# stefanopini/simple-HRNet

Measured on AMD Instinct MI355X. Metric: person-crops/sec HRNet-W48 384x288 (model forward + heat-map decode), higher is better.
Workload: dtype bf16; 1 GPU; HRNet-W48 384x288, batch=256 random crops per GPU, bf16 MFMA (BASELINE configs[2]); global_batch=256, micro_batch=256, lanes_per_gpu=1, parallelism=dp1 (crop sharding, RCCL all-gather of keypoints), weights=random-init seeded (synth_state_dict seed 0), BN stats randomised, engine_switches=

## Files before the change

include/hrnet_mi355.h:

```cpp
#ifndef HRNET_MI355_H
#define HRNET_MI355_H

#include <stddef.h>
#include <stdint.h>

#ifdef __cplusplus
extern "C" {
#endif

typedef struct hrn_ctx *hrn_handle;

enum { HRN_F32 = 0, HRN_BF16 = 1, HRN_F16 = 2 };
enum { HRN_BOX_I32 = 0, HRN_BOX_F32 = 1 };
enum { HRN_T_F32 = 0, HRN_T_I64 = 1 };

typedef struct {
    const char *name;
    const void *data;
    int32_t ndim;
    int64_t dims[4];
    int32_t dtype;
} hrn_tensor_desc;

typedef struct {
// ... 167 lines not shown
                        float *pts_dev, float *heatmaps_dev, void *stream);
int hrn_refine_coords(hrn_handle h, const float *heatmaps_dev, int n, int refine, float *coords_dev, void *stream);

int hrn_nms(int32_t *keep_out, int32_t *num_out, const float *boxes_host, int boxes_num, int boxes_dim,
            float nms_overlap_thresh, int device_id);
int hrn_nms_release(int device_id);
const char *hrn_nms_last_error(void);

int hrn_oks_nms(int32_t *keep_out, int32_t *num_out, const double *kpts, const double *areas, const int32_t *order, int n, int J,
                double thresh, const double *sigmas, double in_vis_thre);
int hrn_soft_oks_nms(int32_t *keep_out, int32_t *num_out, const double *kpts, const double *areas, const double *scores_sorted,
                     const int32_t *order, int n, int J, double thresh, const double *sigmas, double in_vis_thre);
int hrn_pose_similarity(const double *boxes_a, const float *poses_a, int na, const double *boxes_b, const float *poses_b, int nb, int J,
                        float *sim_bbox, float *sim_pose);
int hrn_assignment(const double *cost, int rows, int cols, int32_t *row_to_col);

typedef struct {
    char name[96];
    int32_t c, h, w;
    int32_t conv_index;
} hrn_tap_info;
int hrn_tap_count(hrn_handle h);
int hrn_get_tap_info(hrn_handle h, int index, hrn_tap_info *out);
int hrn_forward_tap(hrn_handle h, const void *images_dev, int n, const char *tap_name, int crop0, int ncrops, int crop_step,
                    float *dst_dev, float *heatmaps_dev, void *stream);

int hrn_conv_count(hrn_handle h);
int hrn_get_conv_info(hrn_handle h, int index, hrn_conv_info *out);
double hrn_flops_per_crop(hrn_handle h);
int64_t hrn_workspace_bytes(hrn_handle h);
int64_t hrn_map_rebuilds(hrn_handle h);
int hrn_launches_per_pass(hrn_handle h);
int hrn_stem_fused(hrn_handle h);
int hrn_conv_compact(hrn_handle h, int index);
const char *hrn_switches(hrn_handle h);
int64_t hrn_debug_pad_violations(hrn_handle h);
int hrn_plan_block_map(hrn_handle h, int group, int n, int reverse, int32_t *blocks, int capacity, int32_t *members,
                       int member_capacity);
int hrn_plan_direct_map(hrn_handle h, int group, int n, int32_t *blocks, int capacity, int32_t *members, int member_capacity,
                        int32_t *pixels_per_tile);
int hrn_plan_s2_map(hrn_handle h, int group, int n, int32_t *blocks, int capacity, int32_t *parts, int part_capacity,
                    int32_t *active);
int hrn_profile_pass(hrn_handle h, const void *images_dev, int n, float *conv_ms, int conv_ms_len,
                     float *other_ms , void *stream);
const char *hrn_version(void);

#ifdef __cplusplus
}
#endif
#endif
```

simple-hrnet_amd/_lib.py:

```python
from __future__ import annotations

import ctypes
import os
import shutil
import subprocess
from typing import List

_HERE = os.path.dirname(os.path.abspath(__file__))
CSRC = os.path.join(_HERE, "csrc")
INCLUDE = os.path.join(os.path.dirname(_HERE), "include")
LIB_PATH = os.path.join(_HERE, "libhrnet_mi355.so")
if os.environ.get("HRN_LIB_TAG"):
    LIB_PATH = LIB_PATH.replace(".so", "_%s.so" % os.environ["HRN_LIB_TAG"])
SOURCES = ["kernels.hip", "conv3x3_lds.hip", "conv_s2.hip", "stem_fused.hip", "conv3x3_f32.hip", "bottleneck_chain.hip", "prepath.hip", "warp.hip", "nms.hip", "postproc.cpp", "hrnet_mi355.cpp",
           "decode.hip",
           "score.hip",
           "draw.hip",
           "track.hip",
           "pose_nms.hip",
           "letterbox.hip",
           "assoc.hip",
           "conv3x3_lds_f16.hip", "conv_s2_f16.hip", "bottleneck_chain_f16.hip"]
HEADERS = [os.path.join(CSRC, "kernels.h"), os.path.join(CSRC, "dt16.h"), os.path.join(CSRC, "argmax.h"), os.path.join(CSRC, "conv3x3_n96.inc"), os.path.join(CSRC, "conv3x3_lds.inc"),
           os.path.join(CSRC, "conv_s2.inc"), os.path.join(CSRC, "bottleneck_chain.inc"), os.path.join(INCLUDE, "hrnet_mi355.h")]
# ... 207 lines not shown
    "hrn_yuv_from_bgr": (ctypes.c_int, [ctypes.c_int, ctypes.c_int, _P, ctypes.c_int, _P]),
    "hrn_crop_geometry": (ctypes.c_int, [_P, ctypes.c_int, ctypes.c_int, _P, ctypes.c_int, ctypes.c_int, ctypes.c_int, ctypes.c_int, _P, _P]),
    "hrn_crop_geometry_last_error": (ctypes.c_char_p, []),
    "hrn_pose_boxes": (ctypes.c_int, [_P, ctypes.c_int, ctypes.c_int, _P, ctypes.c_int, ctypes.c_float, ctypes.c_int, ctypes.c_double,
                                      ctypes.c_double, _P]),
    "hrn_pose_boxes_last_error": (ctypes.c_char_p, []),
    "hrn_boxes_from_poses": (ctypes.c_int, [_P, _P, ctypes.c_int, ctypes.c_int, _P, ctypes.c_int, ctypes.c_float, ctypes.c_int,
                                            ctypes.c_double, ctypes.c_double, _P, _P]),
    "hrn_preprocess_frames_dev": (ctypes.c_int, [_P, ctypes.POINTER(Frame), ctypes.c_int, _P, ctypes.c_int, _P, ctypes.c_int, ctypes.c_int,
                                                 _P, _P, _P, _P]),
    "hrn_preprocess_frames_yuv_dev": (ctypes.c_int, [_P, ctypes.POINTER(YuvFrameC), ctypes.c_int, _P, ctypes.c_int, _P, ctypes.c_int,
                                                     ctypes.c_int, _P, _P, _P, _P]),
    "hrn_forward_flip_tta": (ctypes.c_int, [_P, _P, ctypes.c_int, _P, ctypes.c_int, ctypes.c_int, _P, _P, _P, _P]),
    "hrn_forward_refined": (ctypes.c_int, [_P, _P, ctypes.c_int, _P, ctypes.c_int, ctypes.c_int, _P, _P, _P]),
    "hrn_refine_coords": (ctypes.c_int, [_P, _P, ctypes.c_int, ctypes.c_int, _P, _P]),
    "hrn_nms": (ctypes.c_int, [_P, _P, _P, ctypes.c_int, ctypes.c_int, ctypes.c_float, ctypes.c_int]),
    "hrn_nms_release": (ctypes.c_int, [ctypes.c_int]),
    "hrn_nms_last_error": (ctypes.c_char_p, []),
    "hrn_oks_nms": (ctypes.c_int, [_P, _P, _P, _P, _P, ctypes.c_int, ctypes.c_int, ctypes.c_double, _P, ctypes.c_double]),
    "hrn_soft_oks_nms": (ctypes.c_int, [_P, _P, _P, _P, _P, _P, ctypes.c_int, ctypes.c_int, ctypes.c_double, _P, ctypes.c_double]),
    "hrn_pose_similarity": (ctypes.c_int, [_P, _P, ctypes.c_int, _P, _P, ctypes.c_int, ctypes.c_int, _P, _P]),
    "hrn_assignment": (ctypes.c_int, [_P, ctypes.c_int, ctypes.c_int, _P]),
    "hrn_tap_count": (ctypes.c_int, [_P]),
    "hrn_get_tap_info": (ctypes.c_int, [_P, ctypes.c_int, ctypes.POINTER(TapInfo)]),
    "hrn_forward_tap": (ctypes.c_int, [_P, _P, ctypes.c_int, ctypes.c_char_p, ctypes.c_int, ctypes.c_int, ctypes.c_int, _P, _P, _P]),
    "hrn_conv_count": (ctypes.c_int, [_P]),
    "hrn_get_conv_info": (ctypes.c_int, [_P, ctypes.c_int, ctypes.POINTER(ConvInfo)]),
    "hrn_flops_per_crop": (ctypes.c_double, [_P]),
    "hrn_workspace_bytes": (ctypes.c_int64, [_P]),
    "hrn_map_rebuilds": (ctypes.c_int64, [_P]),
    "hrn_launches_per_pass": (ctypes.c_int, [_P]),
    "hrn_switches": (ctypes.c_char_p, [_P]),
    "hrn_stem_fused": (ctypes.c_int, [_P]),
    "hrn_conv_compact": (ctypes.c_int, [_P, ctypes.c_int]),
    "hrn_debug_pad_violations": (ctypes.c_int64, [_P]),
    "hrn_plan_block_map": (ctypes.c_int, [_P, ctypes.c_int, ctypes.c_int, ctypes.c_int, _P, ctypes.c_int, _P, ctypes.c_int]),
    "hrn_plan_direct_map": (ctypes.c_int, [_P, ctypes.c_int, ctypes.c_int, _P, ctypes.c_int, _P, ctypes.c_int, _P]),
    "hrn_plan_s2_map": (ctypes.c_int, [_P, ctypes.c_int, ctypes.c_int, _P, ctypes.c_int, _P, ctypes.c_int, _P]),
    "hrn_profile_pass": (ctypes.c_int, [_P, _P, ctypes.c_int, ctypes.POINTER(ctypes.c_float), ctypes.c_int,
                                        ctypes.POINTER(ctypes.c_float), _P]),
    "hrn_version": (ctypes.c_char_p, []),
}

_lib = None


def load(auto_build: bool = True) -> ctypes.CDLL:
    global _lib
    if _lib is not None:
        return _lib
    if auto_build and needs_build():
        build()
    lib = ctypes.CDLL(LIB_PATH)
    for name, (res, args) in SYMBOLS.items():
        fn = getattr(lib, name)
        fn.restype = res
        fn.argtypes = args
    _lib = lib
    return lib


def header_symbols() -> List[str]:
    import re

    text = open(os.path.join(INCLUDE, "hrnet_mi355.h")).read()
    text = re.sub(r"/\*.*?\*/", "", text, flags=re.S)
# ... 2 lines not shown
```

simple-hrnet_amd/csrc/ctx_plan.inc:

```
    int new_tensor(int ch, int h, int w) {
        Tensor t;
        t.c = ch, t.h = h, t.w = w, t.wp = w + 1, t.hp = h + 1, t.hpwp = t.wp * t.hp;
        for (size_t i = 0; i < buffers.size(); ++i)
            if (!buffers[i].in_use && buffers[i].c == ch && buffers[i].h == h && buffers[i].w == w) {
                t.buf = (int)i;
                break;
            }
        if (t.buf < 0) {
            Buffer b;
            b.c = ch, b.h = h, b.w = w;
            b.lead_rows = (size_t)t.wp + 1;
            b.rows = b.lead_rows + (size_t)max_batch * t.hpwp + t.wp + 1 + kConvBlockRows;
            b.bytes = (size_t)align_up((int64_t)(b.rows * ch * esize), 256);
            buffers.push_back(b);
            t.buf = (int)buffers.size() - 1;
        }
        buffers[t.buf].in_use = true;
        tensors.push_back(t);
        return (int)tensors.size() - 1;
    }
    void release(int t) { buffers[tensors[t].buf].in_use = false; }

    int default_nr(int cout, int stride) const {
        int nr = (cout % 64 == 0) ? 4 : (cout % 48 == 0) ? 3 : 2;
// ... 371 lines not shown
        if (is16() && !disable_stem_fuse && !disable_stem_mfma && stem_fused_fits(tensors[x].wp, W)) {
            stem_fuse = true;
            convs.back().w2_image = true;
            stemf = S2Group();
            stemf.conv_idx = {(int)convs.size() - 1};
            for (int t = 0; t < 2; ++t) {
                if (stemf.probs.empty()) {
                    stemf.probs.push_back(S2Group::Prob());
                    stemf.probs[0].in_t = stem_out_t;
                    stemf.probs[0].rows = 1, stemf.probs[0].tiles_per_image = tensors[x].h;
                }
                stemf.probs[0].parts.push_back({(int)convs.size() - 1, t});
            }
        }
        release(stem_out_t);
        char buf[96];
        x = add_layer1(x, 4);
        std::vector<int> xs;
        xs.push_back(add_conv("transition1.0.0", "transition1.0.1", x, c, 3, 1, 1, -1, false));
        xs.push_back(add_conv("transition1.1.0.0", "transition1.1.0.1", x, 2 * c, 3, 2, 1, -1, false));
        emit_convs({(int)convs.size() - 2, (int)convs.size() - 1});
        release(x);
        add_stage("stage2.0", xs, 2);
        xs.push_back(add_conv("transition2.2.0.0", "transition2.2.0.1", xs[1], 4 * c, 3, 2, 1));
        for (int m = 0; m < 4; ++m) {
            snprintf(buf, sizeof buf, "stage3.%d", m);
            add_stage(buf, xs, 3);
        }
        xs.push_back(add_conv("transition3.3.0.0", "transition3.3.0.1", xs[2], 8 * c, 3, 2, 1));
        add_stage("stage4.0", xs, 4);
        add_stage("stage4.1", xs, 4);
        add_stage("stage4.2", xs, 1);
        head_in_t = xs[0];
        ops.push_back({OP_HEAD, 0});
        ops.push_back({OP_DECODE, 0});

        layout_blob();
    }

    void index_taps() {
        taps.clear();
        auto add = [&](const std::string &name, int tensor, int op, int conv) {
            for (TapPoint &t : taps)
                if (t.name == name) {
                    t.op = op;
                    return;
                }
            taps.push_back(TapPoint{name, tensor, op, conv});
        };
        for (size_t oi = 0; oi < ops.size(); ++oi) {
            const Op &op = ops[oi];
            switch (op.kind) {
                case OP_STEM:
                case OP_STEM7: add("stem", stem_out_t, (int)oi, -1); break;
                case OP_MAXPOOL: add("maxpool", pool_out_t, (int)oi, -1); break;
                case OP_CONV: add(convs[op.idx].conv, convs[op.idx].out_t, (int)oi, op.idx); break;
                case OP_CONV3_GROUP:
                    for (int ci : groups[op.idx].conv_idx) add(convs[ci].conv, convs[ci].out_t, (int)oi, ci);
                    break;
                case OP_CONV_GROUP:
                    for (int ci : dgroups[op.idx].conv_idx) add(convs[ci].conv, convs[ci].out_t, (int)oi, ci);
                    break;
                case OP_S2_GROUP:
                    for (int ci : s2groups[op.idx].conv_idx) add(convs[ci].conv, convs[ci].out_t, (int)oi, ci);
                    break;
                case OP_CHAIN:
// ... 43 lines not shown
```

simple-hrnet_amd/csrc/ctx_run.inc:

```
    struct Timing {
        std::vector<hipEvent_t> ev;
    };

    bool run_pass(const float *images, int nb, const void *boxes, int box_dtype, float *pts, float *heatmaps,
                  hipStream_t s, Timing *tm, int flip = 0, const TapReq *tap = nullptr, int refine = RF_NONE) {
        if (tm && !hip_ok(hipEventRecord(tm->ev[0], s), "hipEventRecord")) return false;
        const bool fused_stem = stem_fuse && !(tap && tap->op == 0);
        for (size_t oi = 0; oi < ops.size(); ++oi) {
            const bool rev = alternate && (oi & 1);
            hipError_t e = hipSuccess;
            if (fused_stem && oi == 0)
                e = exec_stem_fused(images, nb, s, flip);
            else if (!(fused_stem && (int)oi == stem_conv2_op))
                e = exec_op(ops[oi], rev, images, nb, boxes, box_dtype, pts, heatmaps, s, flip, refine);
            if (!hip_ok(e, "kernel launch")) return false;
            if (tap && tap->op == (int)oi) {
                const Tensor &t = tensors[tap->tensor];
                TapArgs a;
                a.in = row0(tap->tensor), a.dst = tap->dst;
                a.c = t.c, a.h = t.h, a.w = t.w, a.wp = t.wp, a.hpwp = t.hpwp;
                a.crop0 = tap->crop0, a.ncrops = tap->ncrops, a.crop_step = tap->crop_step;
                if (!hip_ok(launch_tap(dtype, a, s), "tap launch")) return false;
            }
            if (tm && !hip_ok(hipEventRecord(tm->ev[oi + 1], s), "hipEventRecord")) return false;
        }
        return true;
    }

    hipError_t exec_stem_fused(const float *images, int nb, hipStream_t s, int flip) {
        S2Group &g = stemf;
        bool hit;
        MapSlot *sl = find_slot(g.slot, nb, &hit);
        hipError_t e = slot_ready(sl, hit, s);
        if (e != hipSuccess) return e;
        if (!hit) {
            sl->nblocks = s2_blocks(g, nb, &g.map_host);
            if (sl->nblocks > g.map_capacity) return hipErrorInvalidValue;
            memcpy(sl->pin, g.map_host.data(), (size_t)sl->nblocks * sizeof(int2));
            e = hipMemcpyAsync(sl->dev, sl->pin, (size_t)sl->nblocks * sizeof(int2), hipMemcpyHostToDevice, s);
            if (e == hipSuccess) e = hipEventRecord(sl->landed, s);
            if (e != hipSuccess) return e;
            sl->nb = nb;
            ++map_builds;
        }
        const Tensor &t = tensors[stem_out_t];
        StemArgs a;
        a.images = images, a.out = nullptr;
        a.w = nullptr, a.bias = (const float *)(blob + stem_b_off), a.wp = (const void *)(blob + stem_wp_off);
        a.n = nb, a.H = H, a.W = W;
        a.out_h = t.h, a.out_w = t.w, a.out_wp = t.wp, a.out_hpwp = t.hpwp;
        a.flip = flip;
        return launch_stem_fused(dtype, s2probs_dev + g.prob_first, sl->dev, sl->nblocks, a, s);
    }

    hipError_t exec_op(const Op &op, bool rev, const float *images, int nb, const void *boxes, int box_dtype, float *pts,
                       float *heatmaps, hipStream_t s, int flip, int refine) {
        hipError_t e = hipSuccess;
        switch (op.kind) {
        case OP_STEM: {
            const Tensor &t = tensors[stem_out_t];
            StemArgs a;
            a.images = images, a.out = row0(stem_out_t);
            a.w = (const float *)(blob + stem_w_off), a.bias = (const float *)(blob + stem_b_off);
            a.wp = (is16() && !disable_stem_mfma) ? (const void *)(blob + stem_wp_off) : nullptr;
            a.n = nb, a.H = H, a.W = W;
            a.out_h = t.h, a.out_w = t.w, a.out_wp = t.wp, a.out_hpwp = t.hpwp;
            a.flip = flip;
            e = launch_stem(dtype, a, s);
            break;
        }
        case OP_STEM7: {
            const Tensor &t = tensors[stem_out_t];
            Stem7Args a;
            a.images = images, a.out = row0(stem_out_t);
            a.w = (const float *)(blob + stem_w_off), a.bias = (const float *)(blob + stem_b_off);
            a.wp = (is16() && !disable_stem_mfma) ? (const void *)(blob + stem_wp_off) : nullptr;
            a.n = nb, a.H = H, a.W = W;
            a.out_h = t.h, a.out_w = t.w, a.out_wp = t.wp, a.out_hpwp = t.hpwp;
            a.flip = flip;
            e = launch_stem7(dtype, a, s);
            break;
        }
        case OP_MAXPOOL: {
            const Tensor &ti = tensors[pool_in_t], &to = tensors[pool_out_t];
            PoolArgs a;
            a.in = row0(pool_in_t), a.out = row0(pool_out_t);
            a.c = to.c, a.n = nb, a.in_wp = ti.wp, a.in_hpwp = ti.hpwp;
            a.out_h = to.h, a.out_w = to.w, a.out_wp = to.wp, a.out_hpwp = to.hpwp;
            e = launch_maxpool(dtype, a, s);
// ... 114 lines not shown
            a.m = nb * to.hpwp, a.h = to.h, a.w = to.w, a.wp = to.wp, a.hpwp = to.hpwp, a.rev = rev, a.max_blocks = chain_blocks;
            e = dtype == HRN_F16 ? launch_bottleneck_chain_f16(a, s) : launch_bottleneck_chain(a, s);
            break;
        }
        case OP_FUSE: {
            FuseGroupArgs ga;
            ga.nf = fuses[op.idx].group;
            for (int k = 0; k < ga.nf; ++k) {
                const FuseOp &f = fuses[op.idx + k];
                const Tensor &to = tensors[f.out_t];
                FuseArgs &a = ga.f[k];
                a.nterms = f.nterms;
                for (int i = 0; i < f.nterms; ++i) {
                    const Tensor &tt = tensors[f.term_t[i]];
                    a.t[i].ptr = row0(f.term_t[i]), a.t[i].shift = f.shift[i];
                    a.t[i].wp = tt.wp, a.t[i].hpwp = tt.hpwp;
                }
                for (int i = f.nterms; i < 4; ++i) a.t[i] = FuseTerm{nullptr, 0, 0, 0};
                a.out = row0(f.out_t), a.c = to.c, a.h = to.h, a.w = to.w, a.wp = to.wp, a.hpwp = to.hpwp;
                a.m = nb * to.hpwp, a.rev = rev;
            }
            e = ga.nf == 1 ? launch_fuse(dtype, ga.f[0], s) : launch_fuse_group(dtype, ga, s);
            break;
        }
        case OP_HEAD: {
            const Tensor &t = tensors[head_in_t];
            HeadArgs a;
            a.in = row0(head_in_t);
            a.wgt = (const float *)(blob + head_w_off), a.bias = (const float *)(blob + head_b_off);
            a.wimg = (is16() && !disable_head_mfma) ? (const void *)(blob + head_wp_off) : nullptr;
            a.heatmaps = heatmaps, a.part_val = part_val, a.part_idx = part_idx;
            a.n = nb, a.c = t.c, a.joints = joints, a.h = t.h, a.w = t.w, a.wp = t.wp, a.hpwp = t.hpwp;
            a.slabs = head_slabs_for(nb), a.slab_px = head_px_for(nb);
            e = launch_head(dtype, a, s);
            break;
        }
        case OP_DECODE: {
            if (!pts) break;
            const Tensor &t = tensors[head_in_t];
            DecodeArgs a{};
            a.part_val = part_val, a.part_idx = part_idx, a.heatmaps = heatmaps, a.boxes = boxes;
            a.box_is_float = box_dtype == HRN_BOX_F32, a.pts = pts;
            a.n = nb, a.joints = joints, a.h = t.h, a.w = t.w, a.slabs = head_slabs_for(nb), a.mode = refine;
            e = launch_decode(a, s);
            break;
        }
    }
        return e;
    }

    bool check_forward_args(const void *images, int n, const void *boxes, float *pts, float *heatmaps, bool outputs_optional = false) {
        if (refuse_plan_only()) return false;
        if (!weights_loaded) {
            err = "weights not loaded (call hrn_load_weights or hrn_adopt_weights)";
            return false;
        }
        if (n < 0 || (n > 0 && !images)) {
            err = "bad images / n";
            return false;
        }
        if (!pts && !heatmaps && !outputs_optional) {
            err = "both pts and heatmaps are NULL";
            return false;
        }
        if (pts && !boxes && n > 0) {
            err = "pts requested without boxes";
// ... 5 lines not shown
```

simple-hrnet_amd/csrc/hrnet_mi355.cpp:

```cpp
#include "../../include/hrnet_mi355.h"

#include <hip/hip_runtime.h>

#include <algorithm>
#include <cmath>
#include <cstdio>
#include <cstdlib>
#include <cstring>
#include <map>
#include <memory>
#include <string>
#include <vector>

#include "assoc_math.h"
#include "letterbox_math.h"
#include "pose_nms_math.h"
#include "kernels.h"
#include "track_geometry.h"

namespace {
#include "ctx_types.h"
}

namespace {
// ... 52 lines not shown
    int small_keep_above = env_sw("HRN_SMALL_KEEP") ? atoi(env_sw("HRN_SMALL_KEEP")) : 300;
    bool disable_chain_ds = env_sw("HRN_DISABLE_CHAIN_DS") != nullptr;
    int pre_mode = env_sw("HRN_PRE_MODE") ? atoi(env_sw("HRN_PRE_MODE")) : 1;
    int chain_blocks = env_sw("HRN_CHAIN_BLOCKS") ? atoi(env_sw("HRN_CHAIN_BLOCKS")) : 512;
    bool disable_chain3 = env_sw("HRN_DISABLE_CHAIN3") != nullptr;
    bool direct_wlds = !(env_sw("HRN_DIRECT_WLDS") && atoi(env_sw("HRN_DIRECT_WLDS")) == 0);
    bool direct_xlds = !(env_sw("HRN_DIRECT_XLDS") && atoi(env_sw("HRN_DIRECT_XLDS")) == 0);
    bool conv_xl(const ConvOp &cv) const {
        return direct_xlds && direct_wlds && is16() && cv.k == 3 && cv.stride == 2 && cv.cin % 32 == 0 && !cv.up && cv.res_t < 0 && cv.nr == 6 &&
               cv.kchunks >= 4;
    }
    bool disable_bbf = env_sw("HRN_BBF") && atoi(env_sw("HRN_BBF")) == 0;
    int bbf_tpb_div = env_sw("HRN_BBF_TPB_DIV") ? std::max(1, atoi(env_sw("HRN_BBF_TPB_DIV"))) : 3;
    double bbf_slide_cost = env_sw("HRN_BBF_SLIDE_COST") ? atof(env_sw("HRN_BBF_SLIDE_COST")) : 24600.0;
    int bbf_min_tiles = env_sw("HRN_BBF_MIN_TILES") ? atoi(env_sw("HRN_BBF_MIN_TILES")) : 1100;
    int dgroup_nr_mode = env_sw("HRN_DGROUP_NR") ? atoi(env_sw("HRN_DGROUP_NR")) : 1;
    bool disable_lds32 = env_sw("HRN_DISABLE_LDS32") != nullptr;
    bool disable_n96 = env_sw("HRN_DISABLE_N96") != nullptr;
    bool disable_fgroup = env_sw("HRN_DISABLE_FGROUP") != nullptr;
    bool disable_f32lds = env_sw("HRN_DISABLE_F32LDS") != nullptr;
    int f32_small_slices = env_sw("HRN_F32_SMALL_SLICES") ? atoi(env_sw("HRN_F32_SMALL_SLICES")) : 0;
    std::vector<Conv3Problem> probs_host;
    bool disable_compact = env_sw("HRN_DISABLE_COMPACT") != nullptr;
    double compact_min_pad = env_sw("HRN_COMPACT_MIN_PAD") ? atof(env_sw("HRN_COMPACT_MIN_PAD")) : 0.08;
    bool disable_s2 = env_sw("HRN_DISABLE_S2") != nullptr;
    int s2_min_tiles = env_sw("HRN_S2_MIN_TILES") ? atoi(env_sw("HRN_S2_MIN_TILES")) : 256;
    int s2_target_blocks = env_sw("HRN_S2_BLOCKS") ? std::max(1, atoi(env_sw("HRN_S2_BLOCKS"))) : 256;
    bool disable_stem_mfma = env_sw("HRN_DISABLE_STEM_MFMA") != nullptr;
    bool disable_stem_fuse = env_sw("HRN_DISABLE_STEM_FUSE") != nullptr;
    bool stem_fuse = false;
    int stem_conv2_op = -1;
    S2Group stemf;
    bool disable_head_mfma = env_sw("HRN_DISABLE_HEAD_MFMA") != nullptr;
    bool direct_nr6 = env_sw("HRN_DIRECT_NR6") ? atoi(env_sw("HRN_DIRECT_NR6")) != 0 : true;
    int half_stages_per_block = env_sw("HRN_HALF_STAGES") ? atoi(env_sw("HRN_HALF_STAGES")) : 8;
    bool alternate = env_sw("HRN_ALTERNATE") ? atoi(env_sw("HRN_ALTERNATE")) != 0 : true;
    int block_order = env_sw("HRN_BLOCK_ORDER") ? atoi(env_sw("HRN_BLOCK_ORDER")) : 1;
    int long_factor = env_sw("HRN_LONG_FACTOR") ? atoi(env_sw("HRN_LONG_FACTOR")) : 4;
    double long_share = env_sw("HRN_LONG_SHARE") ? atof(env_sw("HRN_LONG_SHARE")) : 0.85;
    int head_slabs = 1, head_slab_px = 1024;
    static constexpr int kHeadSlabPxSmall = 256;
    int head_slabs_small = 1;
    int head_px_for(int nb) const { return (long)nb * head_slabs >= 192 ? head_slab_px : kHeadSlabPxSmall; }
    int head_slabs_for(int nb) const { return (long)nb * head_slabs >= 192 ? head_slabs : head_slabs_small; }
    float *part_val = nullptr;
    int *part_idx = nullptr;
    uint64_t map_clock = 0;
    int64_t map_builds = 0;
    float *scratch_hm = nullptr;
    float *scratch_heatmaps() {
        if (!scratch_hm && !hip_ok(hipMalloc((void **)&scratch_hm, (size_t)max_batch * joints * (H / 4) * (W / 4) * sizeof(float)),
                                   "hipMalloc(scratch heat-maps)"))
            scratch_hm = nullptr;
        return scratch_hm;
    }
    int64_t workspace_bytes = 0;

#include "ctx_plan.inc"
#include "ctx_memory.inc"
#include "ctx_weights.inc"
#include "ctx_run.inc"
#include "ctx_scratch.inc"
};

namespace {
using CallScope = hrn_ctx::CallScope;
// ... 1224 lines not shown
    if (!h->run_pass((const float *)images_dev, n, nullptr, 0, nullptr, heatmaps_dev, (hipStream_t)stream, nullptr, 0, &req)) return 8;
    return scope.leave() ? 0 : 6;
}

int hrn_conv_count(hrn_handle h) { return h ? (int)h->convs.size() : 0; }

int hrn_get_conv_info(hrn_handle h, int index, hrn_conv_info *out) {
    if (!h || !out || index < 0 || index >= (int)h->convs.size()) return 1;
    const ConvOp &cv = h->convs[index];
    memset(out, 0, sizeof *out);
    snprintf(out->name, sizeof out->name, "%s", cv.conv.c_str());
    out->cin = cv.cin, out->cout = cv.cout, out->ksize = cv.k, out->stride = cv.stride, out->relu = cv.relu;
    out->has_residual = cv.res_t >= 0;
    out->in_h = h->tensors[cv.in_t].h, out->in_w = h->tensors[cv.in_t].w;
    out->out_h = h->tensors[cv.out_t].h, out->out_w = h->tensors[cv.out_t].w;
    out->kpad = cv.kpad, out->nr = cv.nr, out->algo = cv.fuse_with >= 0 || cv.fused_away ? 2 : cv.n96 ? 3 : cv.s2 ? 4 : cv.algo, out->ks = cv.ks;
    out->w_offset = cv.w_off, out->w_bytes = cv.w_bytes, out->b_offset = cv.b_off;
    out->flops = cv.flops;
    return 0;
}

double hrn_flops_per_crop(hrn_handle h) {
    if (!h) return 0;
    double f = 2.0 * 64 * (h->model == 1 ? 147 : 27) * (h->H / 2) * (double)(h->W / 2);
    for (auto &cv : h->convs) f += cv.flops;
    f += 2.0 * h->joints * h->head_c * (h->H / 4) * (double)(h->W / 4);
    return f;
}

int64_t hrn_workspace_bytes(hrn_handle h) { return h ? h->workspace_bytes : 0; }
int64_t hrn_map_rebuilds(hrn_handle h) { return h ? h->map_builds : -1; }
int hrn_launches_per_pass(hrn_handle h) { return h ? (int)h->ops.size() - (h->stem_fuse ? 1 : 0) : 0; }
int hrn_stem_fused(hrn_handle h) { return h && h->stem_fuse ? 1 : 0; }
int hrn_conv_compact(hrn_handle h, int index) { return h && index >= 0 && index < (int)h->convs.size() && h->convs[index].compact ? 1 : 0; }
const char *hrn_switches(hrn_handle h) { return h ? h->switches.c_str() : ""; }

int64_t hrn_debug_pad_violations(hrn_handle h) {
    if (!h || h->plan_only) return -1;
    if (!h->hip_ok(hipSetDevice(h->device), "hipSetDevice")) return -1;
    unsigned long long *cnt = nullptr, host = 0;
    if (!h->hip_ok(hipMalloc((void **)&cnt, sizeof *cnt), "hipMalloc") || !h->hip_ok(hipMemset(cnt, 0, sizeof *cnt), "hipMemset")) return -1;
    bool ok = h->hip_ok(hipDeviceSynchronize(), "hipDeviceSynchronize");
    for (const Buffer &b : h->buffers) {
        if (!ok) break;
        PadCheckArgs a;
        a.buf = b.dev, a.count = cnt, a.rows = (long)b.rows, a.lead_rows = (long)b.lead_rows;
        a.c = b.c, a.h = b.h, a.w = b.w, a.wp = b.w + 1, a.hpwp = (b.h + 1) * (b.w + 1), a.nmax = h->max_batch;
        ok = h->hip_ok(launch_pad_check(h->dtype, a, nullptr), "pad check launch");
    }
    ok = ok && h->hip_ok(hipMemcpy(&host, cnt, sizeof host, hipMemcpyDeviceToHost), "hipMemcpy");
    (void)hipFree(cnt);
    return ok ? (int64_t)host : -1;
}

int hrn_plan_block_map(hrn_handle h, int group, int n, int reverse, int32_t *blocks, int capacity, int32_t *members, int member_capacity) {
    if (!h || n <= 0 || n > h->max_batch) return -1;
    if (group < 0 || group >= (int)h->groups.size()) return -1;
    const Conv3Group &g = h->groups[group];
    std::vector<int2> map;
    std::vector<int> px;
    const int nblocks = h->group_blocks(g, n, &map, reverse != 0, false, &px);
    for (int i = 0; i < nblocks && i < capacity; ++i) {
        const int x = map[i].x, y = map[i].y;
        int32_t *o = blocks + (size_t)i * 6;
        o[0] = x & 0xff, o[1] = (x >> 8) & 0xff, o[2] = x >> 16, o[3] = y & 0x1fffffff, o[4] = px[i],
        o[5] = ((y >> 29) & 1) | (((y >> 30) & 1) << 1);
// ... 123 lines not shown
```

simple-hrnet_amd/csrc/kernels.h:

```cpp
#pragma once
#include <hip/hip_runtime.h>
#include <stdint.h>

#include <atomic>
#include <cstdlib>
#include <cstring>

namespace hrn {

inline hipError_t set_dynamic_lds(const void *func, int bytes, std::atomic<unsigned long long> &done) {
    int dev = 0;
    hipError_t e = hipGetDevice(&dev);
    if (e != hipSuccess) return e;
    const unsigned long long bit = 1ull << (dev & 63);
    if (done.load(std::memory_order_acquire) & bit) return hipSuccess;
    e = hipFuncSetAttribute(func, hipFuncAttributeMaxDynamicSharedMemorySize, bytes);
    if (e == hipSuccess) done.fetch_or(bit, std::memory_order_release);
    return e;
}

inline const char *hrn_env(const char *name) {
    static const bool debug = [] {
        const char *v = getenv("HRN_DEBUG_ENV");
        return v && *v && strcmp(v, "0") != 0;
// ... 179 lines not shown
hipError_t launch_maxpool(int dtype, const PoolArgs &a, hipStream_t s);

struct FuseTerm {
    const void *ptr;
    int shift;
    int wp, hpwp;
};
struct FuseArgs {
    FuseTerm t[4];
    int nterms;
    void *out;
    int c, h, w, wp, hpwp;
    int m;
    int rev;
};

struct FuseGroupArgs {
    FuseArgs f[4];
    int nf;
    int block_end[4];
};
hipError_t launch_fuse_group(int dtype, FuseGroupArgs &g, hipStream_t s);

constexpr int kMaxJoints = 256;
struct HeadArgs {
    const void *in;
    const float *wgt;
    const void *wimg;
    const float *bias;
    float *heatmaps;
    float *part_val;
    int *part_idx;
    int n, c, joints, h, w, wp, hpwp, slabs, slab_px;
};

enum { RF_NONE = 0, RF_QUARTER = 1, RF_DARK = 2 };
struct DecodeArgs {
    const float *part_val;
    const int *part_idx;
    const void *boxes;
    int box_is_float;
    float *pts;
    int n, joints, h, w, slabs, mode;
    const float *heatmaps;
    float *coords;
};
hipError_t launch_decode(const DecodeArgs &a, hipStream_t s);
hipError_t launch_refine_coords(const DecodeArgs &a, hipStream_t s);

struct TtaArgs {
    float *hm;
    const float *hm_flipped;
    float *preds;
    float *maxvals;
    int pair[kMaxJoints];
    int n, joints, h, w, post_processing;
};
hipError_t launch_tta_decode(const TtaArgs &a, hipStream_t s);

struct ScoreJoint {
    int mu_x, mu_y;
    float weight;
    int draw;
};
struct ScoreArgs {
    const float *heatmaps;
// ... 169 lines not shown
```

simple-hrnet_amd/csrc/kernels.hip:

```cpp
#include "kernels.h"
#include "argmax.h"
#include "dt16.h"
#include <stdlib.h>

namespace hrn {

typedef __attribute__((ext_vector_type(8))) __bf16 bf16x8;
typedef __attribute__((ext_vector_type(8))) short s16x8;
typedef __attribute__((ext_vector_type(4))) short s16x4;
typedef __attribute__((ext_vector_type(4))) float f32x4;

__device__ __forceinline__ float bf16_to_f32(unsigned short h) { return __uint_as_float(((unsigned)h) << 16); }
__device__ __forceinline__ unsigned short f32_to_bf16(float f) {
    unsigned u = __float_as_uint(f);
    u += 0x7fffu + ((u >> 16) & 1u);
    return (unsigned short)(u >> 16);
}

constexpr bool is16(int dt) { return dt != DT_F32; }

template <int DT>
struct Tr;
template <>
struct Tr<DT_BF16> {
    using elem = unsigned short;
    using vec = s16x8;
    using out4 = s16x4;
    static constexpr int KC = 32, VEC = 8;
    static __device__ __forceinline__ float ld(elem e) { return bf16_to_f32(e); }
    static __device__ __forceinline__ elem st(float f) { return f32_to_bf16(f); }
};
template <>
struct Tr<DT_F16> {
    using elem = unsigned short;
    using vec = s16x8;
// ... 771 lines not shown
        }
    }
}

hipError_t launch_stem(int dtype, const StemArgs &a, hipStream_t s) {
    const int m = a.n * a.out_hpwp;
    if (m <= 0) return hipSuccess;
    dim3 grid((m + 255) / 256);
    if (dtype == DT_BF16 && a.wp)
        hipLaunchKernelGGL(stem_mfma_kernel<DT_BF16>, grid, dim3(256), 0, s, a);
    else if (dtype == DT_F16 && a.wp)
        hipLaunchKernelGGL(stem_mfma_kernel<DT_F16>, grid, dim3(256), 0, s, a);
    else if (dtype == DT_BF16)
        hipLaunchKernelGGL(stem_kernel<DT_BF16>, grid, dim3(256), 0, s, a);
    else if (dtype == DT_F16)
        hipLaunchKernelGGL(stem_kernel<DT_F16>, grid, dim3(256), 0, s, a);
    else
        hipLaunchKernelGGL(stem_kernel<DT_F32>, grid, dim3(256), 0, s, a);
    return hipGetLastError();
}

template <int DT>
__device__ __forceinline__ void fuse_body(const FuseArgs &p, const long block, const long nblocks) {
    using T = Tr<DT>;
    using vec = typename T::vec;
    const int cvn = p.c / T::VEC;
    const long bid = p.rev ? nblocks - 1 - block : block;
    const long idx = bid * 256 + threadIdx.x;
    const long total = (long)p.m * cvn;
    if (idx >= total) return;
    const int q = (int)(idx / cvn), cv = (int)(idx - (long)q * cvn);
    const int n = q / p.hpwp, rem = q - n * p.hpwp;
    const int r = rem / p.wp, c = rem - r * p.wp;
    float sum[T::VEC];
#pragma unroll
    for (int t = 0; t < 4; ++t) {
        if (t >= p.nterms) break;
        const FuseTerm ft = p.t[t];
        const long row = ft.shift == 0 ? (long)q : (long)n * ft.hpwp + (long)(r >> ft.shift) * ft.wp + (c >> ft.shift);
        const vec v = *(const vec *)((const typename T::elem *)ft.ptr + row * p.c + cv * T::VEC);
#pragma unroll
        for (int e = 0; e < T::VEC; ++e) {
            const float f = T::ld((typename T::elem)v[e]);
            sum[e] = (t == 0) ? f : sum[e] + f;
        }
    }
    vec o;
#pragma unroll
    for (int e = 0; e < T::VEC; ++e) o[e] = T::st(fmaxf(sum[e], 0.f));
    *(vec *)((typename T::elem *)p.out + (long)q * p.c + cv * T::VEC) = o;
}

template <int DT>
__global__ __launch_bounds__(256) void fuse_kernel(const FuseArgs p) {
    fuse_body<DT>(p, blockIdx.x, gridDim.x);
}

template <int DT>
__global__ __launch_bounds__(256) void fuse_group_kernel(const FuseGroupArgs g) {
    int k = 0;
    long first = 0;
#pragma unroll
    for (int i = 0; i < 3; ++i)
        if (k == i && i + 1 < g.nf && (long)blockIdx.x >= g.block_end[i]) first = g.block_end[i], k = i + 1;
    if (k == 0)
        fuse_body<DT>(g.f[0], (long)blockIdx.x - first, (long)g.block_end[0] - first);
    else if (k == 1)
        fuse_body<DT>(g.f[1], (long)blockIdx.x - first, (long)g.block_end[1] - first);
    else if (k == 2)
        fuse_body<DT>(g.f[2], (long)blockIdx.x - first, (long)g.block_end[2] - first);
    else
        fuse_body<DT>(g.f[3], (long)blockIdx.x - first, (long)g.block_end[3] - first);
}

hipError_t launch_fuse(int dtype, const FuseArgs &a, hipStream_t s) {
    const long total = (long)a.m * (a.c / (dtype != DT_F32 ? 8 : 4));
    if (total <= 0) return hipSuccess;
    dim3 grid((unsigned)((total + 255) / 256));
    if (dtype == DT_BF16)
        hipLaunchKernelGGL(fuse_kernel<DT_BF16>, grid, dim3(256), 0, s, a);
    else if (dtype == DT_F16)
        hipLaunchKernelGGL(fuse_kernel<DT_F16>, grid, dim3(256), 0, s, a);
// ... 91 lines not shown
    }
    __syncthreads();
    if (threadIdx.x < jn) {
        const int j = threadIdx.x;
        float v = red_v[j];
        int i = red_i[j];
        for (int w = 1; w < 4; ++w)
            if (better(red_v[w * kJointGroup + j], red_i[w * kJointGroup + j], v, i)) {
                v = red_v[w * kJointGroup + j];
                i = red_i[w * kJointGroup + j];
            }
        p.part_val[((size_t)n * p.joints + j0 + j) * p.slabs + slab] = v;
        p.part_idx[((size_t)n * p.joints + j0 + j) * p.slabs + slab] = i;
    }
}

template <int DT>
__global__ __launch_bounds__(256) void head_kernel(const HeadArgs p) {
    extern __shared__ __attribute__((aligned(16))) float smem[];
    float *red_v = smem + p.joints * p.c;
    head_group<DT>(p, 0, p.joints, false, smem, red_v, (int *)(red_v + 4 * kJointGroup));
}

template <int DT>
__global__ __launch_bounds__(256) void head_groups_kernel(const HeadArgs p) {
    extern __shared__ __attribute__((aligned(16))) float smem[];
    float *red_v = smem + kJointGroup * p.c;
    int *red_i = (int *)(red_v + 4 * kJointGroup);
#pragma unroll 1
    for (int j0 = 0; j0 < p.joints; j0 += kJointGroup)
        head_group<DT>(p, j0, min(kJointGroup, p.joints - j0), j0 != 0, smem, red_v, red_i);
}

template <int DT>
__device__ __forceinline__ void head_mfma_group(const HeadArgs &p, const int j0, const int jn, const bool again, float *red_v, int *red_i) {
    const int lane = threadIdx.x & 63, wave = threadIdx.x >> 6;
    const int li = lane & 15, g = lane >> 4;
    const int slab = blockIdx.x, n = blockIdx.y;
    const int hw = p.h * p.w;
    const int kch = (p.c + 31) >> 5;
    const GLOBAL_AS unsigned short *__restrict__ in = (const GLOBAL_AS unsigned short *)p.in;
    const GLOBAL_AS s16x8 *__restrict__ wimg = (const GLOBAL_AS s16x8 *)p.wimg + (size_t)(j0 >> 4) * kch * 64;
    float bias[8];
#pragma unroll
    for (int f = 0; f < 2; ++f)
#pragma unroll
        for (int r = 0; r < 4; ++r) {
            const int j = f * 16 + 4 * g + r;
            bias[f * 4 + r] = j < jn ? p.bias[j0 + j] : 0.f;
        }
    float bv[8];
    int bi[8];
#pragma unroll
    for (int t = 0; t < 8; ++t) bv[t] = -INFINITY, bi[t] = kNoIdx;

    const int px_per_wave = p.slab_px / 4;
    for (int it = 0; it < px_per_wave / 16; ++it) {
        const int px0 = slab * p.slab_px + wave * px_per_wave + it * 16;
        if (px0 >= hw) break;
        const int px = px0 + li;
        const bool live = px < hw;
        const int pc = live ? px : hw - 1;
        const int r = pc / p.w, c = pc - r * p.w;
        const GLOBAL_AS unsigned short *row = in + ((size_t)n * p.hpwp + r * p.wp + c) * p.c;
        f32x4 acc[2] = {f32x4{0.f, 0.f, 0.f, 0.f}, f32x4{0.f, 0.f, 0.f, 0.f}};
        for (int kc = 0; kc < kch; ++kc) {
            const int k0 = kc * 32 + g * 8;
            s16x8 x = {};
            if (k0 < p.c) x = *(const GLOBAL_AS s16x8 *)(row + k0);
#pragma unroll
            for (int f = 0; f < 2; ++f) acc[f] = mma<DT>(wimg[(f * kch + kc) * 64 + lane], x, acc[f]);
        }
#pragma unroll
        for (int f = 0; f < 2; ++f)
#pragma unroll
            for (int q = 0; q < 4; ++q) {
                const int t = f * 4 + q, j = f * 16 + 4 * g + q;
                const float v = acc[f][q] + bias[t];
                if (live && j < jn) {
                    if (p.heatmaps) p.heatmaps[((size_t)n * p.joints + j0 + j) * hw + px] = v;
                    if (takes(v, bv[t], bi[t])) bv[t] = v, bi[t] = px;
                }
            }
    }
    if (again) __syncthreads();
#pragma unroll
    for (int t = 0; t < 8; ++t) {
        float v = bv[t];
        int i = bi[t];
#pragma unroll
        for (int off = 8; off > 0; off >>= 1) {
            const float ov = __shfl_xor(v, off);
            const int oi = __shfl_xor(i, off);
            if (better(ov, oi, v, i)) v = ov, i = oi;
        }
        const int j = (t >> 2) * 16 + 4 * g + (t & 3);
        if (li == 0 && j < kJointGroup) red_v[wave * kJointGroup + j] = v, red_i[wave * kJointGroup + j] = i;
    }
    __syncthreads();
    if (threadIdx.x < jn) {
        const int j = threadIdx.x;
        float v = red_v[j];
        int i = red_i[j];
        for (int w = 1; w < 4; ++w)
            if (better(red_v[w * kJointGroup + j], red_i[w * kJointGroup + j], v, i)) {
                v = red_v[w * kJointGroup + j];
                i = red_i[w * kJointGroup + j];
            }
        p.part_val[((size_t)n * p.joints + j0 + j) * p.slabs + slab] = v;
        p.part_idx[((size_t)n * p.joints + j0 + j) * p.slabs + slab] = i;
    }
}

template <int DT>
__global__ __launch_bounds__(256) void head_mfma_kernel(const HeadArgs p) {
    __shared__ float red_v[4 * kJointGroup];
    __shared__ int red_i[4 * kJointGroup];
    head_mfma_group<DT>(p, 0, p.joints, false, red_v, red_i);
}

template <int DT>
__global__ __launch_bounds__(256) void head_mfma_groups_kernel(const HeadArgs p) {
    __shared__ float red_v[4 * kJointGroup];
    __shared__ int red_i[4 * kJointGroup];
#pragma unroll 1
    for (int j0 = 0; j0 < p.joints; j0 += kJointGroup)
        head_mfma_group<DT>(p, j0, min(kJointGroup, p.joints - j0), j0 != 0, red_v, red_i);
}

hipError_t launch_head(int dtype, const HeadArgs &a, hipStream_t s) {
    if (a.n <= 0) return hipSuccess;
    if (a.joints <= 0 || a.joints > kMaxJoints) return hipErrorInvalidValue;
    const bool groups = a.joints > kJointGroup;
    dim3 grid(a.slabs, a.n);
    if (dtype != DT_F32 && a.wimg && a.slab_px % 64 == 0) {
        if (dtype == DT_F16)
            hipLaunchKernelGGL(groups ? head_mfma_groups_kernel<DT_F16> : head_mfma_kernel<DT_F16>, grid, dim3(256), 0, s, a);
        else
            hipLaunchKernelGGL(groups ? head_mfma_groups_kernel<DT_BF16> : head_mfma_kernel<DT_BF16>, grid, dim3(256), 0, s, a);
        return hipGetLastError();
    }
    const int staged = groups ? kJointGroup : a.joints;
    const size_t shm = sizeof(float) * ((size_t)staged * a.c + 4 * kJointGroup) + sizeof(int) * 4 * kJointGroup;
    if (dtype == DT_BF16)
        hipLaunchKernelGGL(groups ? head_groups_kernel<DT_BF16> : head_kernel<DT_BF16>, grid, dim3(256), shm, s, a);
    else if (dtype == DT_F16)
        hipLaunchKernelGGL(groups ? head_groups_kernel<DT_F16> : head_kernel<DT_F16>, grid, dim3(256), shm, s, a);
    else
        hipLaunchKernelGGL(groups ? head_groups_kernel<DT_F32> : head_kernel<DT_F32>, grid, dim3(256), shm, s, a);
    return hipGetLastError();
}

template <int DT>
__global__ __launch_bounds__(256) void tap_kernel(const TapArgs p) {
    using T = Tr<DT>;
    const long idx = (long)blockIdx.x * 256 + threadIdx.x;
    const long per = (long)p.c * p.h * p.w;
    if (idx >= per * p.ncrops) return;
    const int n = (int)(idx / per);
    const int rem = (int)(idx - (long)n * per);
    const int ch = rem / (p.h * p.w), px = rem - ch * (p.h * p.w);
    const int r = px / p.w, c = px - r * p.w;
    const typename T::elem *in = (const typename T::elem *)p.in;
    p.dst[idx] = T::ld(in[((size_t)(p.crop0 + n * p.crop_step) * p.hpwp + (size_t)r * p.wp + c) * p.c + ch]);
}

hipError_t launch_tap(int dtype, const TapArgs &a, hipStream_t s) {
// ... 44 lines not shown
```

simple-hrnet_amd/native.py:

```python
from __future__ import annotations

import contextlib
import ctypes
import math
from typing import Dict, List, Optional, Sequence, Tuple, Union

import numpy as np
import torch

from . import _lib
from .frames import (PIX_FORMATS, YUV_MATRICES, YUV_RANGES, Frames, YuvFrame, _check_frame, _frame_kind, as_tensor,
                     device_tensor, frame_stack, host_array, host_bytes)
from .palettes import bgr_to_yuv_colors, embedded_palette, find_palette

DTYPES = {"fp32": 0, "f32": 0, "float32": 0, torch.float32: 0, "bf16": 1, "bfloat16": 1, torch.bfloat16: 1,
          "fp16": 2, "f16": 2, "float16": 2, "half": 2, torch.float16: 2}
DTYPE_NAMES = {0: "fp32", 1: "bf16", 2: "fp16"}
REFINE_MODES = {None: 0, "quarter": 1, "dark": 2}


def refine_code(refine) -> int:
    if not (refine is None or isinstance(refine, str)) or refine not in REFINE_MODES:
        raise ValueError("refine must be None, 'quarter' or 'dark', got %r" % (refine,))
    return REFINE_MODES[refine]
# ... 1003 lines not shown
        h, w = self.resolution
        hm = torch.empty((n, self.nof_joints, h // 4, w // 4), dtype=torch.float32, device=x.device) if return_heatmaps else None
        self._launch("hrn_forward_tap", x.data_ptr(), n, name.encode(), int(crop0), int(ncrops), int(crop_step), dst.data_ptr(),
                     hm.data_ptr() if hm is not None else None)
        return (dst, hm) if return_heatmaps else dst

    def conv_infos(self) -> List[_lib.ConvInfo]:
        out = []
        for i in range(self._lib.hrn_conv_count(self._h)):
            ci = _lib.ConvInfo()
            rc = self._lib.hrn_get_conv_info(self._h, i, ctypes.byref(ci))
            self._check(rc, "hrn_get_conv_info")
            out.append(ci)
        return out

    def flops_per_crop(self) -> float:
        return float(self._lib.hrn_flops_per_crop(self._h))

    def workspace_bytes(self) -> int:
        return int(self._lib.hrn_workspace_bytes(self._h))

    def map_rebuilds(self) -> int:
        return int(self._lib.hrn_map_rebuilds(self._h))

    def launches_per_pass(self) -> int:
        return int(self._lib.hrn_launches_per_pass(self._h))

    def conv_compact(self, index: int) -> bool:
        return bool(self._lib.hrn_conv_compact(self._h, index))

    def stem_fused(self) -> bool:
        return bool(self._lib.hrn_stem_fused(self._h))

    def pad_violations(self) -> int:
        return int(self._lib.hrn_debug_pad_violations(self._h))

    def switches(self) -> str:
        return self._lib.hrn_switches(self._h).decode()

    def profile_pass(self, images: torch.Tensor):
        x = self._images_ptr(images)
        n = min(x.shape[0], self.max_batch)
        nconv = self._lib.hrn_conv_count(self._h)
        conv_ms = (ctypes.c_float * nconv)()
        other = (ctypes.c_float * 4)()
        self._launch("hrn_profile_pass", x.data_ptr(), n, conv_ms, nconv, other)
        return list(conv_ms), dict(zip(("stem", "fuse", "head", "decode"), list(other)))


class MultiDeviceHRNet:

    def __init__(self, devices: Sequence[int], c: int = 48, nof_joints: int = 17, resolution: Tuple[int, int] = (384, 288),
                 dtype="bf16", max_batch: int = 32, model_name: str = "HRNet"):
        from concurrent.futures import ThreadPoolExecutor

        if len(devices) < 1:
            raise ValueError("at least one device")
        self.devices = [int(d) for d in devices]
        self.nets = [NativeHRNet(c, nof_joints, resolution, dtype, max_batch=max_batch, device=d, model_name=model_name)
                     for d in self.devices]
        self.streams = [torch.cuda.Stream(torch.device("cuda", d)) for d in self.devices]
        self.pool = ThreadPoolExecutor(max_workers=len(self.devices), thread_name_prefix="hrn-dev")
        first = self.nets[0]
        self.c, self.nof_joints, self.resolution = first.c, first.nof_joints, first.resolution
        self.dtype, self.max_batch, self.model_name = first.dtype, first.max_batch, first.model_name
        self.device_index = first.device_index
# ... 152 lines not shown
```

Measured before the change: 11380 crops/s.

## Fuse final stage-4 branch sum+ReLU into the MFMA heat-map head kernel

The last fuse op of stage 4 (summing the four upsampled branches into the 48-channel high-res tensor, then ReLU) is skipped. Instead the MFMA head kernel recomputes that sum on the fly from the four branch tensors while loading its input. Weights are held in registers when there are only one or two K-chunks. This removes one kernel launch plus a full write and re-read of the fused tensor. In exchange, the head now does gather-style reads from the lower-resolution branches and uses more registers.

```diff
diff --git a/include/hrnet_mi355.h b/include/hrnet_mi355.h
--- a/include/hrnet_mi355.h
+++ b/include/hrnet_mi355.h
@@ -223,6 +223,7 @@
 int64_t hrn_map_rebuilds(hrn_handle h);
 int hrn_launches_per_pass(hrn_handle h);
 int hrn_stem_fused(hrn_handle h);
+int hrn_head_fused(hrn_handle h);
 int hrn_conv_compact(hrn_handle h, int index);
 const char *hrn_switches(hrn_handle h);
 int64_t hrn_debug_pad_violations(hrn_handle h);
diff --git a/simple-hrnet_amd/_lib.py b/simple-hrnet_amd/_lib.py
--- a/simple-hrnet_amd/_lib.py
+++ b/simple-hrnet_amd/_lib.py
@@ -263,6 +263,7 @@
     "hrn_launches_per_pass": (ctypes.c_int, [_P]),
     "hrn_switches": (ctypes.c_char_p, [_P]),
     "hrn_stem_fused": (ctypes.c_int, [_P]),
+    "hrn_head_fused": (ctypes.c_int, [_P]),
     "hrn_conv_compact": (ctypes.c_int, [_P, ctypes.c_int]),
     "hrn_debug_pad_violations": (ctypes.c_int64, [_P]),
     "hrn_plan_block_map": (ctypes.c_int, [_P, ctypes.c_int, ctypes.c_int, ctypes.c_int, _P, ctypes.c_int, _P, ctypes.c_int]),
diff --git a/simple-hrnet_amd/csrc/ctx_plan.inc b/simple-hrnet_amd/csrc/ctx_plan.inc
--- a/simple-hrnet_amd/csrc/ctx_plan.inc
+++ b/simple-hrnet_amd/csrc/ctx_plan.inc
@@ -427,6 +427,11 @@
         add_stage("stage4.1", xs, 4);
         add_stage("stage4.2", xs, 1);
         head_in_t = xs[0];
+        if (is16() && !disable_head_fuse && !disable_head_mfma && joints <= 32 && ops.back().kind == OP_FUSE &&
+            fuses[ops.back().idx].group == 1 && fuses[ops.back().idx].out_t == head_in_t && fuses[ops.back().idx].nterms == 4) {
+            head_fuse = true;
+            head_fuse_op = (int)ops.size() - 1;
+        }
         ops.push_back({OP_HEAD, 0});
         ops.push_back({OP_DECODE, 0});
 
diff --git a/simple-hrnet_amd/csrc/ctx_run.inc b/simple-hrnet_amd/csrc/ctx_run.inc
--- a/simple-hrnet_amd/csrc/ctx_run.inc
+++ b/simple-hrnet_amd/csrc/ctx_run.inc
@@ -6,13 +6,14 @@
                   hipStream_t s, Timing *tm, int flip = 0, const TapReq *tap = nullptr, int refine = RF_NONE) {
         if (tm && !hip_ok(hipEventRecord(tm->ev[0], s), "hipEventRecord")) return false;
         const bool fused_stem = stem_fuse && !(tap && tap->op == 0);
+        const bool fused_head = head_fuse && !(tap && tap->op == head_fuse_op);
         for (size_t oi = 0; oi < ops.size(); ++oi) {
             const bool rev = alternate && (oi & 1);
             hipError_t e = hipSuccess;
             if (fused_stem && oi == 0)
                 e = exec_stem_fused(images, nb, s, flip);
-            else if (!(fused_stem && (int)oi == stem_conv2_op))
-                e = exec_op(ops[oi], rev, images, nb, boxes, box_dtype, pts, heatmaps, s, flip, refine);
+            else if (!(fused_stem && (int)oi == stem_conv2_op) && !(fused_head && (int)oi == head_fuse_op))
+                e = exec_op(ops[oi], rev, images, nb, boxes, box_dtype, pts, heatmaps, s, flip, refine, fused_head);
             if (!hip_ok(e, "kernel launch")) return false;
             if (tap && tap->op == (int)oi) {
                 const Tensor &t = tensors[tap->tensor];
@@ -54,7 +55,7 @@
     }
 
     hipError_t exec_op(const Op &op, bool rev, const float *images, int nb, const void *boxes, int box_dtype, float *pts,
-                       float *heatmaps, hipStream_t s, int flip, int refine) {
+                       float *heatmaps, hipStream_t s, int flip, int refine, bool fused_head = false) {
         hipError_t e = hipSuccess;
         switch (op.kind) {
         case OP_STEM: {
@@ -235,6 +236,14 @@
             a.heatmaps = heatmaps, a.part_val = part_val, a.part_idx = part_idx;
             a.n = nb, a.c = t.c, a.joints = joints, a.h = t.h, a.w = t.w, a.wp = t.wp, a.hpwp = t.hpwp;
             a.slabs = head_slabs_for(nb), a.slab_px = head_px_for(nb);
+            if (fused_head) {
+                const FuseOp &f = fuses[ops[head_fuse_op].idx];
+                a.nterms = f.nterms;
+                for (int i = 0; i < f.nterms; ++i) {
+                    const Tensor &tt = tensors[f.term_t[i]];
+                    a.t[i] = FuseTerm{row0(f.term_t[i]), f.shift[i], tt.wp, tt.hpwp};
+                }
+            }
             e = launch_head(dtype, a, s);
             break;
         }
diff --git a/simple-hrnet_amd/csrc/fuse_sum.h b/simple-hrnet_amd/csrc/fuse_sum.h
--- /dev/null
+++ b/simple-hrnet_amd/csrc/fuse_sum.h
@@ -0,0 +1,30 @@
+#pragma once
+
+#include "kernels.h"
+
+namespace hrn {
+
+template <class T, int NT>
+__device__ __forceinline__ typename T::vec fuse_value(const FuseTerm (&terms)[4], const int p_nterms, const int cs, const long q, const int n,
+                                                      const int r, const int c, const int ch) {
+    using vec = typename T::vec;
+    float sum[T::VEC];
+#pragma unroll
+    for (int t = 0; t < 4; ++t) {
+        if (NT ? t >= NT : t >= p_nterms) break;
+        const FuseTerm ft = terms[t];
+        const long row = ft.shift == 0 ? q : (long)n * ft.hpwp + (long)(r >> ft.shift) * ft.wp + (c >> ft.shift);
+        const vec v = *(const vec *)((const typename T::elem *)ft.ptr + row * cs + ch);
+#pragma unroll
+        for (int e = 0; e < T::VEC; ++e) {
+            const float f = T::ld((typename T::elem)v[e]);
+            sum[e] = (t == 0) ? f : sum[e] + f;
+        }
+    }
+    vec o;
+#pragma unroll
+    for (int e = 0; e < T::VEC; ++e) o[e] = T::st(fmaxf(sum[e], 0.f));
+    return o;
+}
+
+}
diff --git a/simple-hrnet_amd/csrc/hrnet_mi355.cpp b/simple-hrnet_amd/csrc/hrnet_mi355.cpp
--- a/simple-hrnet_amd/csrc/hrnet_mi355.cpp
+++ b/simple-hrnet_amd/csrc/hrnet_mi355.cpp
@@ -108,6 +108,9 @@
     int stem_conv2_op = -1;
     S2Group stemf;
     bool disable_head_mfma = env_sw("HRN_DISABLE_HEAD_MFMA") != nullptr;
+    bool disable_head_fuse = env_sw("HRN_DISABLE_HEAD_FUSE") != nullptr;
+    bool head_fuse = false;
+    int head_fuse_op = -1;
     bool direct_nr6 = env_sw("HRN_DIRECT_NR6") ? atoi(env_sw("HRN_DIRECT_NR6")) != 0 : true;
     int half_stages_per_block = env_sw("HRN_HALF_STAGES") ? atoi(env_sw("HRN_HALF_STAGES")) : 8;
     bool alternate = env_sw("HRN_ALTERNATE") ? atoi(env_sw("HRN_ALTERNATE")) != 0 : true;
@@ -1398,6 +1401,7 @@
 int64_t hrn_map_rebuilds(hrn_handle h) { return h ? h->map_builds : -1; }
 int hrn_launches_per_pass(hrn_handle h) { return h ? (int)h->ops.size() - (h->stem_fuse ? 1 : 0) : 0; }
 int hrn_stem_fused(hrn_handle h) { return h && h->stem_fuse ? 1 : 0; }
+int hrn_head_fused(hrn_handle h) { return h && h->head_fuse ? 1 : 0; }
 int hrn_conv_compact(hrn_handle h, int index) { return h && index >= 0 && index < (int)h->convs.size() && h->convs[index].compact ? 1 : 0; }
 const char *hrn_switches(hrn_handle h) { return h ? h->switches.c_str() : ""; }
 
diff --git a/simple-hrnet_amd/csrc/kernels.h b/simple-hrnet_amd/csrc/kernels.h
--- a/simple-hrnet_amd/csrc/kernels.h
+++ b/simple-hrnet_amd/csrc/kernels.h
@@ -235,6 +235,8 @@
     float *part_val;
     int *part_idx;
     int n, c, joints, h, w, wp, hpwp, slabs, slab_px;
+    FuseTerm t[4] = {};
+    int nterms = 0;
 };
 
 enum { RF_NONE = 0, RF_QUARTER = 1, RF_DARK = 2 };
diff --git a/simple-hrnet_amd/csrc/kernels.hip b/simple-hrnet_amd/csrc/kernels.hip
--- a/simple-hrnet_amd/csrc/kernels.hip
+++ b/simple-hrnet_amd/csrc/kernels.hip
@@ -1,6 +1,7 @@
 #include "kernels.h"
 #include "argmax.h"
 #include "dt16.h"
+#include "fuse_sum.h"
 #include <stdlib.h>
 
 namespace hrn {
@@ -838,22 +839,7 @@
     const int q = (int)(idx / cvn), cv = (int)(idx - (long)q * cvn);
     const int n = q / p.hpwp, rem = q - n * p.hpwp;
     const int r = rem / p.wp, c = rem - r * p.wp;
-    float sum[T::VEC];
-#pragma unroll
-    for (int t = 0; t < 4; ++t) {
-        if (t >= p.nterms) break;
-        const FuseTerm ft = p.t[t];
-        const long row = ft.shift == 0 ? (long)q : (long)n * ft.hpwp + (long)(r >> ft.shift) * ft.wp + (c >> ft.shift);
-        const vec v = *(const vec *)((const typename T::elem *)ft.ptr + row * p.c + cv * T::VEC);
-#pragma unroll
-        for (int e = 0; e < T::VEC; ++e) {
-            const float f = T::ld((typename T::elem)v[e]);
-            sum[e] = (t == 0) ? f : sum[e] + f;
-        }
-    }
-    vec o;
-#pragma unroll
-    for (int e = 0; e < T::VEC; ++e) o[e] = T::st(fmaxf(sum[e], 0.f));
+    const vec o = fuse_value<T, 0>(p.t, p.nterms, p.c, (long)q, n, r, c, cv * T::VEC);
     *(vec *)((typename T::elem *)p.out + (long)q * p.c + cv * T::VEC) = o;
 }
 
@@ -1011,7 +997,7 @@
         head_group<DT>(p, j0, min(kJointGroup, p.joints - j0), j0 != 0, smem, red_v, red_i);
 }
 
-template <int DT>
+template <int DT, bool FUSED = false, int KCH = 0>
 __device__ __forceinline__ void head_mfma_group(const HeadArgs &p, const int j0, const int jn, const bool again, float *red_v, int *red_i) {
     const int lane = threadIdx.x & 63, wave = threadIdx.x >> 6;
     const int li = lane & 15, g = lane >> 4;
@@ -1033,6 +1019,13 @@
 #pragma unroll
     for (int t = 0; t < 8; ++t) bv[t] = -INFINITY, bi[t] = kNoIdx;
 
+    s16x8 wreg[2][KCH > 0 ? KCH : 1];
+    if constexpr (FUSED && KCH > 0) {
+#pragma unroll
+        for (int f = 0; f < 2; ++f)
+#pragma unroll
+            for (int kc = 0; kc < KCH; ++kc) wreg[f][kc] = wimg[(f * KCH + kc) * 64 + lane];
+    }
     const int px_per_wave = p.slab_px / 4;
     for (int it = 0; it < px_per_wave / 16; ++it) {
         const int px0 = slab * p.slab_px + wave * px_per_wave + it * 16;
@@ -1043,10 +1036,27 @@
         const int r = pc / p.w, c = pc - r * p.w;
         const GLOBAL_AS unsigned short *row = in + ((size_t)n * p.hpwp + r * p.wp + c) * p.c;
         f32x4 acc[2] = {f32x4{0.f, 0.f, 0.f, 0.f}, f32x4{0.f, 0.f, 0.f, 0.f}};
+        if constexpr (FUSED && KCH > 0) {
+            s16x8 xs[KCH];
+#pragma unroll
+            for (int kc = 0; kc < KCH; ++kc) {
+                const int k0 = kc * 32 + g * 8;
+                xs[kc] = fuse_value<Tr<DT>, 4>(p.t, 4, p.c, (long)n * p.hpwp + r * p.wp + c, n, r, c, min(k0, p.c - 8));
+                if (k0 >= p.c) xs[kc] = s16x8{};
+            }
+#pragma unroll
+            for (int kc = 0; kc < KCH; ++kc)
+#pragma unroll
+                for (int f = 0; f < 2; ++f) acc[f] = mma<DT>(wreg[f][kc], xs[kc], acc[f]);
+        } else
         for (int kc = 0; kc < kch; ++kc) {
             const int k0 = kc * 32 + g * 8;
             s16x8 x = {};
-            if (k0 < p.c) x = *(const GLOBAL_AS s16x8 *)(row + k0);
+            if constexpr (FUSED) {
+                if (k0 < p.c) x = fuse_value<Tr<DT>, 4>(p.t, 4, p.c, (long)n * p.hpwp + r * p.wp + c, n, r, c, k0);
+            } else {
+                if (k0 < p.c) x = *(const GLOBAL_AS s16x8 *)(row + k0);
+            }
 #pragma unroll
             for (int f = 0; f < 2; ++f) acc[f] = mma<DT>(wimg[(f * kch + kc) * 64 + lane], x, acc[f]);
         }
@@ -1098,6 +1108,24 @@
     head_mfma_group<DT>(p, 0, p.joints, false, red_v, red_i);
 }
 
+template <int DT, int KCH>
+__global__ __launch_bounds__(256) void head_mfma_fused_kernel(const HeadArgs p) {
+    __shared__ float red_v[4 * kJointGroup];
+    __shared__ int red_i[4 * kJointGroup];
+    head_mfma_group<DT, true, KCH>(p, 0, p.joints, false, red_v, red_i);
+}
+
+template <int DT>
+static void launch_head_fused(const HeadArgs &a, dim3 grid, hipStream_t s) {
+    const int kch = (a.c + 31) >> 5;
+    if (kch == 1)
+        hipLaunchKernelGGL((head_mfma_fused_kernel<DT, 1>), grid, dim3(256), 0, s, a);
+    else if (kch == 2)
+        hipLaunchKernelGGL((head_mfma_fused_kernel<DT, 2>), grid, dim3(256), 0, s, a);
+    else
+        hipLaunchKernelGGL((head_mfma_fused_kernel<DT, 0>), grid, dim3(256), 0, s, a);
+}
+
 template <int DT>
 __global__ __launch_bounds__(256) void head_mfma_groups_kernel(const HeadArgs p) {
     __shared__ float red_v[4 * kJointGroup];
@@ -1112,6 +1140,15 @@
     if (a.joints <= 0 || a.joints > kMaxJoints) return hipErrorInvalidValue;
     const bool groups = a.joints > kJointGroup;
     dim3 grid(a.slabs, a.n);
+    if (a.nterms) {
+        if (a.nterms != 4 || groups || dtype == DT_F32 || !a.wimg || a.slab_px % 64 != 0) return hipErrorInvalidValue;
+        if (a.c < 8 || a.c % 8) return hipErrorInvalidValue;
+        if (dtype == DT_F16)
+            launch_head_fused<DT_F16>(a, grid, s);
+        else
+            launch_head_fused<DT_BF16>(a, grid, s);
+        return hipGetLastError();
+    }
     if (dtype != DT_F32 && a.wimg && a.slab_px % 64 == 0) {
         if (dtype == DT_F16)
             hipLaunchKernelGGL(groups ? head_mfma_groups_kernel<DT_F16> : head_mfma_kernel<DT_F16>, grid, dim3(256), 0, s, a);
diff --git a/simple-hrnet_amd/native.py b/simple-hrnet_amd/native.py
--- a/simple-hrnet_amd/native.py
+++ b/simple-hrnet_amd/native.py
@@ -1059,6 +1059,9 @@
     def stem_fused(self) -> bool:
         return bool(self._lib.hrn_stem_fused(self._h))
 
+    def head_fused(self) -> bool:
+        return bool(self._lib.hrn_head_fused(self._h))
+
     def pad_violations(self) -> int:
         return int(self._lib.hrn_debug_pad_violations(self._h))
 
```

Result: no change. 11350 crops/s (-0.2%).
